# normallytangent/dune-eigensolver

Hardware: AMD Instinct MI355X
Metric: Lanczos iters/sec + achieved SpMV HBM GB/s, 3D Poisson 256^3 (higher is better)
Workload: dtype f64

## Files before the change

dune-eigensolver_amd/csrc/api.cpp:

```cpp
#include <algorithm>
#include <cmath>
#include <cstdlib>
#include <cstring>
#include <atomic>
#include <mutex>
#include <random>
#include <thread>

#include "internal.h"

using namespace eigmi;

namespace {

struct DeviceGuard {
  int prev = -1;
  explicit DeviceGuard(int dev)
  {
    if (hipGetDevice(&prev) != hipSuccess) prev = -1;
    if (prev != dev) EIG_HIP(hipSetDevice(dev));
  }
  ~DeviceGuard()
  {
    if (prev >= 0) (void)hipSetDevice(prev);
// ... 1628 lines not shown
    info->ncols = A->nb_cols * A->bc;
    info->row_begin = A->row_begin * A->br;
    info->window = A->window;
    info->own_offset = A->own_offset;
    info->nnzb = A->nnzb;
    info->nnzb_padded = A->nnzb_padded;
    info->nslices = A->nslices;
    info->br = A->br;
    info->bc = A->bc;
    info->halo_recv = A->halo_recv;
    info->halo_send = A->halo_send;
    info->device_bytes = A->device_bytes;
    info->stencil_slices = A->n_stencil_slices;
    info->rows_per_lane = A->R;
    info->sym_offsets = A->sym_val ? A->sym_nd : 0;
    info->sym_arrays = A->sym_val ? A->sym_nup : 0;
    info->sym_mask_bytes = A->sym_val ? A->sym_mask_bytes : 0;
    info->sym_uniform = (A->sym_val && A->sym_uniform && !(A->kflags & EIG_MAT_NO_UNIFORM))
                            ? (A->sym_geo ? 2 : 1)
                            : 0;
    info->sym_geo = A->sym_val && A->sym_geo ? 1 : 0;
    info->march_variant = march_variant(*A, true);
    info->march_variant_mv = march_variant(*A, false);
  });
}

extern "C" int eig_lanczos_kernel_info(eig_mat_t A, int fused, char *name, int name_len, int64_t *bytes)
{
  return guard(A ? A->ctx : nullptr, [&] {
    EIG_CHECK(A && bytes && (name || name_len == 0), EIG_ERR_ARG, "eig_lanczos_kernel_info: null argument");
    std::string nm;
    i64 b = 0;
    lanczos_kernel_info(*A, fused != 0, nm, b);
    *bytes = b;
    if (name_len > 0)
    {
      const size_t k = std::min<size_t>(nm.size(), (size_t)name_len - 1);
      std::memcpy(name, nm.data(), k);
      name[k] = 0;
    }
  });
}

extern "C" int eig_mat_kernel_info(eig_mat_t A, int op, char *name, int name_len)
{
  return guard(A ? A->ctx : nullptr, [&] {
// ... 549 lines not shown
```

dune-eigensolver_amd/csrc/drivers.cpp:

```cpp
#include <algorithm>
#include <complex>
#include <cmath>
#include <cstdlib>
#include <cstring>
#include <numeric>
#include <string>
#include <vector>

#include "internal.h"

using namespace eigmi;

namespace {

bool distributed(const eig_mat_s &A) { return A.ctx->distributed(); }

struct PinnedDoubles {
  double *p = nullptr, *dev = nullptr;
  explicit PinnedDoubles(size_t n)
  {
    EIG_HIP(hipHostMalloc(reinterpret_cast<void **>(&p), (n ? n : 1) * sizeof(double), hipHostMallocMapped));
    EIG_HIP(hipHostGetDevicePointer(reinterpret_cast<void **>(&dev), p, 0));
  }
  ~PinnedDoubles()
// ... 1686 lines not shown
      }
      launch_fused_tail(ws->lb->st, ws->L, ctx->stream);
    }
    else
      launch_beta_tail(ws->lb->st, ws->k, ctx->stream);
    EIG_HIP(hipStreamSynchronize(ctx->stream));
    check_step_exchange(*ws);
    if (k) *k = ws->k;
    if (alpha_host && ws->k > 0)
      EIG_HIP(hipMemcpy(alpha_host, ws->lb->st.alpha, ws->k * sizeof(double), hipMemcpyDeviceToHost));
    if (beta_host) EIG_HIP(hipMemcpy(beta_host, ws->lb->st.beta, (ws->k + 1) * sizeof(double), hipMemcpyDeviceToHost));
  });
}

extern "C" int eig_lanczos_info(eig_lanczos_t ws, int *steps, int *launches)
{
  return guard(ws ? ws->A->ctx : nullptr, [&] {
    EIG_CHECK(ws, EIG_ERR_ARG, "eig_lanczos_info: null workspace");
    if (steps) *steps = ws->k;
    if (launches) *launches = ws->fused ? ws->L : ws->k;
  });
}

extern "C" int eig_lanczos_destroy(eig_lanczos_t ws)
{
  if (!ws) return EIG_OK;
  (void)hipSetDevice(ws->A->ctx->device);
  (void)hipStreamSynchronize(ws->A->ctx->stream);
  delete ws;
  return EIG_OK;
}

extern "C" int eig_lanczos_run(eig_mat_t A, int steps, const double *u0, unsigned seed, int flags, double *alpha_host,
                               double *beta_host, eig_timing *timing)
{
  eig_lanczos_t ws = nullptr;
  const int kind = EIG_LANCZOS_FUSED | EIG_LANCZOS_PIPELINED;
  int rc = eig_lanczos_create_ex(A, steps, u0, seed, flags & kind, &ws);
  if (rc != EIG_OK) return rc;
  rc = eig_lanczos_step(ws, steps, flags & ~kind, timing);
  if (rc == EIG_OK) rc = eig_lanczos_tridiag(ws, nullptr, alpha_host, beta_host);
  eig_lanczos_destroy(ws);
  return rc;
}

extern "C" int eig_lanczos_solve(eig_mat_t A, int nev, int ncv, int which, unsigned seed, double *eval_host,
// ... 99 lines not shown
```

dune-eigensolver_amd/csrc/internal.h:

```cpp
#pragma once
#include <hip/hip_runtime.h>
#include <rccl/rccl.h>

#include <complex>
#include <condition_variable>
#include <cstdint>
#include <mutex>
#include <new>
#include <stdexcept>
#include <string>
#include <memory>
#include <vector>

#include "../../include/eigmi.h"

namespace eigmi {

typedef int64_t i64;
typedef int32_t i32;
typedef uint64_t u64;

struct Error : std::runtime_error {
  int code;
  Error(int c, const std::string &m) : std::runtime_error(m), code(c) {}
// ... 233 lines not shown
  double *fred;
  int *ctl;
  double *aux;
  double *mu2;
  double *pn;
};
enum { kFusedModeStep = 0, kFusedModePost = 1, kFusedModeHalt = 2 };
struct FusedLaunch {
  LanczosState st;
  int L;
  int force;
  int xch = 0;
};
enum { kXchPublish = 2 };
void launch_lanczos_fused(const eig_mat_s &A, const double *P, double *Pout, const FusedLaunch &fl,
                          const i32 *slices, i64 first, i64 count, const double *carry, double *out, int ticket,
                          hipStream_t s, ReduceWS red);
void launch_lanczos_pipe(const eig_mat_s &A, double *T, double *UZ, const double *S, const FusedLaunch &fl,
                         double *out, hipStream_t s, ReduceWS red);
void launch_fused_tail(const LanczosState &st, int L, hipStream_t s);
bool march_geometry(const eig_mat_s &A, i64 &D, int chunk = 64);
bool march_split_active(const eig_mat_s &A);
int march_variant(const eig_mat_s &A, bool fused);
extern const i32 kMarchInteriorTag;
bool box_prepare(const eig_mat_s &A);
inline bool box_spmm_applies(const eig_mat_s &A, i64 m)
{
  return m > 0 && m % 8 == 0 && box_prepare(A) && (A.box_ctab != nullptr || m % 32 == 0);
}
int box_cols(const eig_mat_s &A);
bool launch_box_spmm(const eig_mat_s &A, i64 m, const double *X, double *Y, hipStream_t s);
bool launch_box_spmm_dot(const eig_mat_s &A, i64 m, const double *X, double *Y, double *dp, ReduceWS red,
                         hipStream_t s);
bool launch_box_spmm_dot_gram(const eig_mat_s &A, i64 m, const double *X, double *Y, double *dp, double *gram,
                              ReduceWS red, hipStream_t s, unsigned *zero_word = nullptr);
bool launch_spmm_march_dot_gram(const eig_mat_s &A, i64 m, const double *X, double *Y, double *dp, double *gram,
                                ReduceWS red, hipStream_t s, unsigned *zero_word = nullptr);
unsigned *mgs_lookahead_barrier(eig_ctx_t ctx);
bool launch_spmm_dot_gram_mv8(const eig_mat_s &A, i64 m, const double *X, double *Y, double *dp, double *gram,
                              hipStream_t s, ReduceWS red);
bool launch_spmm_march_dot(const eig_mat_s &A, i64 m, const double *X, double *Y, double *dp, ReduceWS red,
                           hipStream_t s);
bool launch_box_cheb(const eig_mat_s &M, i64 m, const double *Xk, double *Xold, const double *B, const double *dinv,
                     double omega, double gamma, hipStream_t s, double *Xnew = nullptr);
void box_invalidate(eig_mat_s &A);
bool launch_box_resid(const eig_mat_s &A, i64 m, const double *X, const double *B, double *R, hipStream_t s);
// ... 217 lines not shown
```

dune-eigensolver_amd/csrc/k_spmv.hip:

```cpp
#include "internal.h"
#include "march_variants.h"
#include "reduce_dev.h"
#include "xch_dev.h"

namespace eigmi {

constexpr int kWaves = kStreamThreads / 64;

template <int R>
struct Vec;
template <>
struct Vec<1> {
  typedef double d;
  typedef i32 i;
};
template <>
struct Vec<2> {
  typedef double d __attribute__((ext_vector_type(2)));
  typedef i32 i __attribute__((ext_vector_type(2)));
};
template <>
struct Vec<4> {
  typedef double d __attribute__((ext_vector_type(4)));
  typedef i32 i __attribute__((ext_vector_type(4)));
};

// ... 1071 lines not shown
  }
  double v[3] = {d, q2, m2};
  fused_finish<2>(v, partials, ticket, tot, out, carry, fa);
}

struct MarchPlan {
  i64 D;
  i64 zb;
  i64 nplanes;
  i64 mrows;
  int ncol;
  int nseg;
  i32 dn, dq;
  const double *Un, *Uq;
  double cD, c0, c1, cn, cq;
  int gx, gy, gz, gz0;
  int uni;
  int tstore;
  signed char kj[27];
  const double *pack;
  int cache;
  int lines;
  int down;
};
template <class T>
__device__ __forceinline__ void march_store(const MarchPlan &mp, T v, T *p)
{
  if (mp.tstore)
    *p = v;
  else
    __builtin_nontemporal_store(v, p);
}

template <int PF, bool PG, class X, class EPI>
__device__ __forceinline__ void march_rows_geo(const SellB1 &A, const MarchPlan &mp, i64 own, int lane, int wave,
                                               const X &x, EPI &epi)
{
  typedef typename X::raw raw;
  const SymImg &S = A.sym;
  const int xl = (int)A.xlast, D = (int)mp.D, own32 = (int)own;
  const int nd = S.nd;
  const int item = (int)swizzled_block() * kWaves + wave;
  if (item >= mp.ncol * mp.nseg) return;
  const int col = item % mp.ncol, seg = item / mp.ncol;
  const int z0 = (int)(mp.zb + seg * mp.nplanes / mp.nseg), z1 = (int)(mp.zb + (seg + 1) * mp.nplanes / mp.nseg);
  auto cx = [&](int g) -> unsigned { return g < 0 ? 0u : (unsigned)(g > xl ? xl : g); };
// ... 251 lines not shown
  };
  static_assert(!PG || NS % 2 == 0, "gather prefetch: an even number of bodies per trip");
  static_assert(!VPF || NS % 2 == 0, "value prefetch: an even number of bodies per trip");
  int z = z0;
  for (; z + NS - 1 < z1; z += NS)
  {
#pragma unroll
    for (int k = 0; k < NS; ++k)
      body(z + k, sl[k], sl[(k + 1) % NS], sl[(k + PF + 1) % NS], gs[PG ? k & 1 : 0], gs[PG ? (k + 1) & 1 : 1],
           vs[VPF ? k & 1 : 0], vs[VPF ? (k + 1) & 1 : 1]);
  }
#pragma unroll
  for (int k = 0; k < NS - 1; ++k)
    if (z + k < z1)
      body(z + k, sl[k], sl[(k + 1) % NS], sl[(k + PF + 1) % NS], gs[PG ? k & 1 : 0], gs[PG ? (k + 1) & 1 : 1],
           vs[VPF ? k & 1 : 0], vs[VPF ? (k + 1) & 1 : 1]);
}

constexpr bool kMarch2lDefault = true;
constexpr bool kMarch2lSerpentine = true;
constexpr bool march_down_variant(int uni) { return uni == 22 || uni == 23; }
template <int UNI>
constexpr bool kMarchDownBody = march_down_variant(UNI);

template <bool DOWN, class X, class EPI, class PRE>
__device__ __forceinline__ void march_rows_geo2_2l(const SellB1 &A, const MarchPlan &mp, i64 own, int lane, int wave,
                                                   X x, EPI &epi, PRE &pre)
{
  typedef typename X::raw raw;
  constexpr unsigned SZ = sizeof(raw);
  const int D = (int)mp.D, own32 = (int)own, gx = mp.gx;
  const int item = (int)swizzled_block() * kWaves + wave;
  if (item >= mp.ncol * mp.nseg) return;
  const int col2 = item % mp.ncol, seg = item / mp.ncol;
  const int xcols = gx / 64;
  const int x0 = (col2 % xcols) * 64, y0 = (col2 / xcols) * 2;
  const int z0 = (int)(mp.zb + seg * mp.nplanes / mp.nseg), z1 = (int)(mp.zb + (seg + 1) * mp.nplanes / mp.nseg);
  const unsigned nbytes = (unsigned)(A.xlast + 1) * SZ;
  const __amdgpu_buffer_rsrc_t rs = __builtin_amdgcn_make_buffer_rsrc(const_cast<void *>(x.ptr()), 0, (int)nbytes, 0x00020000);
  const __amdgpu_buffer_rsrc_t r0 = __builtin_amdgcn_make_buffer_rsrc(const_cast<void *>(x.ptr()), 0, 0, 0x00020000);
  const bool has_n = mp.dn && y0 > 0, has_q = mp.dq && y0 + 2 < mp.gy;
  const __amdgpu_buffer_rsrc_t rn = has_n ? rs : r0, rq = has_q ? rs : r0;
  constexpr unsigned kOut = 0x80000000u;
  const unsigned eoff = lane == 0 ? (x0 > 0 ? 0u - SZ : kOut) : lane == 63 ? (x0 + 64 < gx ? SZ : kOut) : kOut;
  const unsigned dnb = (unsigned)mp.dn * SZ, dqb = (unsigned)mp.dq * SZ, Db = (unsigned)D * SZ, nxb = (unsigned)gx * SZ;
  int w = own32 + y0 * gx + x0 + lane + z0 * D;
  unsigned vo = (unsigned)w * SZ;
  const int zg0 = z0 + mp.gz0;
  const SymImg &S = A.sym;
  const dpair *P01 = reinterpret_cast<const dpair *>(mp.pack), *P23 = P01 + S.ld;
  const bool le = lane == 0 && x0 > 0;
  if constexpr (DOWN)
  {
    auto row = [&](double amD, double vmD, double an, double vn, double am, double vl, double a0, double vc, double a1,
                   double vr, double aq, double vq, double prodD) {
      double acc = 0.0;
      acc += amD * vmD;
      acc += an * vn;
      acc += am * vl;
      acc += a0 * vc;
      acc += a1 * vr;
      acc += aq * vq;
      acc += prodD;
      return acc;
    };
    w += (z1 - 1 - z0) * D;
    vo = (unsigned)w * SZ;
    const bool above = z1 + mp.gz0 < mp.gz;
    raw pu0{}, pu1{};
    if (above)
    {
      bload(rs, vo + Db, pu0);
      bload(rs, vo + nxb + Db, pu1);
    }
// ... 323 lines not shown

template <int UNI>
constexpr MarchTraits kTraits = march_traits(UNI);
template <int UNI>
constexpr bool kWholePlanes = kTraits<UNI>.whole_planes();
template <int UNI>
constexpr bool kUniformValues = kTraits<UNI>.values == kMarchUniform;

template <class MT, int KC, bool SPAN1, int UNI, class X, class EPI, class PRE = MarchNoPre>
__device__ __forceinline__ void march_rows(const SellB1 &A, const MarchPlan &mp, i64 own, int lane, int wave,
                                           const X &x, EPI &epi, PRE &&pre = PRE{})
{
  static_assert(kTraits<UNI>.valid, "not a march variant (march_variants.h)");
  static_assert(kTraits<UNI>.any_head() ||
                    (SPAN1 == kTraits<UNI>.span1() && (int)sizeof(MT) == kTraits<UNI>.mask_bytes()),
                "march variant instantiated with another template head than its traits name");
  if constexpr (kTraits<UNI>.family == kMarchKuhn)
  {
    march_rows_kuhn<kTraits<UNI>.kp, kTraits<UNI>.lx>(A, mp, own, lane, wave, x, epi, pre);
    return;
  }
  else if constexpr (kTraits<UNI>.family == kMarchGeo2L2)
  {
    if constexpr (kMarchDownBody<UNI>)
      if (mp.down)
      {
        march_rows_geo2_2l<true>(A, mp, own, lane, wave, x, epi, pre);
        return;
      }
    march_rows_geo2_2l<false>(A, mp, own, lane, wave, x, epi, pre);
    return;
  }
  else if constexpr (kTraits<UNI>.family == kMarchGeo2)
  {
    march_rows_geo2<kTraits<UNI>.pf, kTraits<UNI>.pg, kTraits<UNI>.val>(A, mp, own, lane, wave, x, epi, pre);
    return;
  }
  else if constexpr (kTraits<UNI>.family == kMarchGeo)
  {
    march_rows_geo<kTraits<UNI>.pf, kTraits<UNI>.pg>(A, mp, own, lane, wave, x, epi);
    return;
  }
  constexpr bool GEO = kTraits<UNI>.geo_masks;
  typedef typename X::raw raw;
  const SymImg &S = A.sym;
  const int xl = (int)A.xlast, D = (int)mp.D, ldl = (int)(S.ld - 1), own32 = (int)own, mrows = (int)mp.mrows;
// ... 815 lines not shown
    mp.gz = A.sym_gz;
    mp.gz0 = A.sym_gz0;
  }
  if (A.sym_uniform)
  {
    const int kD = A.sym_nd - 1;
    int kz = -1, k1 = -1;
    for (int k = 0; k < A.sym_nd; ++k)
    {
      if (A.sym_off[k] == 0) kz = k;
      if (A.sym_off[k] == 1) k1 = k;
    }
    mp.cD = A.sym_uc[A.sym_dj[kD]];
    mp.c0 = kz >= 0 ? A.sym_uc[A.sym_dj[kz]] : 0.0;
    mp.c1 = k1 >= 0 ? A.sym_uc[A.sym_dj[k1]] : 0.0;
    mp.cn = klo > 1 ? A.sym_uc[A.sym_dj[1]] : 0.0;
    mp.cq = khi < A.sym_nd - 1 ? A.sym_uc[A.sym_dj[khi]] : 0.0;
  }
  mp.uni = uni;
  mp.pack = pack && T.needs_pack() ? sym_pack_prepare(A) : nullptr;
  mp.tstore = fused && T.geo2_path() && (vectors_fit_mall(A) || (A.tune_cache & 1));
  mp.cache = A.tune_cache;
  mp.down = march_down_variant(uni) && (A.tune_cache & 24) == 16;
  mp.lines = A.tune_march_lines == 4 && T.line_groups && mp.gx % 64 == 0 &&
                     mp.gx > 0 && mp.gy % 4 == 0 && (i64)mp.gx * mp.gy == D
                 ? 4
                 : 0;
  mp.zb = zb;
  mp.nplanes = nplanes;
  mp.mrows = A.nslices * 64;
  mp.ncol = (int)items_per_run;
  mp.nseg = (int)nseg;
  return mp;
}

int march_variant(const eig_mat_s &A, bool fused)
{
  if (A.br != 1 || A.bc != 1) return -1;
  const MarchPlan mp = march_plan(A, image_mode(A), 0, -1, fused);
  return mp.nseg > 0 ? mp.uni : -1;
}

const i32 kMarchInteriorTag = 0;

void march_prepare(const eig_mat_s &A)
{
  if (A.br != 1 || A.bc != 1) return;
  const int mode = image_mode(A);
  for (bool fused : {false, true})
  {
    (void)march_plan(A, mode, 0, -1, fused, 64, true);
    if (A.mz1 > A.mz0) (void)march_plan(A, mode, A.mz0, A.mz1, fused, 64, true);
  }
}

bool march_split_active(const eig_mat_s &A)
{
  return A.mz1 > A.mz0 && march_plan(A, image_mode(A), A.mz0, A.mz1).nseg > 0;
}

static MarchPlan launch_plan(const eig_mat_s &A, int mode, const i32 *slices, i64 first, i64 count,
                             bool fused = false)
{
// ... 138 lines not shown
    fa.mb = A.ctx->mbox->dev;
  }
#define EIG_LFB(B_)                                                                                          \
  if (A.br == B_)                                                                                            \
  {                                                                                                          \
    hipLaunchKernelGGL((k_lanczos_fused_blk<B_>),                                                            \
                       dim3(grid_for_slices(k_lanczos_fused_blk<B_>, count, A.ctx->num_cu)),                 \
                       dim3(kStreamThreads), 0, s, A.nb_rows, A.slice_ptr, slices, first, count, A.val, A.col, \
                       reinterpret_cast<const dpair *>(P), reinterpret_cast<dpair *>(Pout), fa, out, carry,   \
                       red.partials, red.ticket(ticket));                                                    \
    return;                                                                                                  \
  }
  EIG_LFB(2) EIG_LFB(3) EIG_LFB(4)
#undef EIG_LFB
  if (!carry)
  {
    const int mode = image_mode(A);
    MarchPlan mp = launch_plan(A, mode, slices, first, count, true);
    if (mp.nseg > 0)
    {
      if (march_down_variant(mp.uni) && ((A.tune_cache & 24) == 24 || (kMarch2lSerpentine && !(A.tune_cache & 24))))
        mp.down = fl.L & 1;
      march_launch(MarchDispatch{}, A, mode, mp.uni, [&](auto mt, auto span1, auto uni) {
        hipLaunchKernelGGL((k_lanczos_fused_march<decltype(mt), span1(), uni()>), dim3(march_grid(mp)),
                           dim3(kStreamThreads), 0, s, A.nb_rows, A.own_offset, sell_b1(A), mp,
                           reinterpret_cast<const dpair *>(P), reinterpret_cast<dpair *>(Pout), fa, out, red.partials,
                           red.ticket(ticket));
      });
      return;
    }
  }
#define EIG_LF_(R_, M_, CPF_)                                                                                 \
  hipLaunchKernelGGL((k_lanczos_fused_b1<R_, M_, CPF_>),                                                     \
                     dim3(grid_for_slices(k_lanczos_fused_b1<R_, M_, CPF_>, count, A.ctx->num_cu)),           \
                     dim3(kStreamThreads), 0, s, A.nb_rows, A.own_offset, sell_b1(A), slices, first, count,      \
                     reinterpret_cast<const dpair *>(P), reinterpret_cast<dpair *>(Pout), fa, out, carry,        \
                     red.partials, red.ticket(ticket))
#define EIG_LF(R_, M_)                                                                                        \
  do                                                                                                          \
  {                                                                                                           \
    if (sell_cpf(A, true) && (M_ == kExplicit || M_ == kMixed)) EIG_LF_(R_, M_, true);                        \
    else EIG_LF_(R_, M_, false);                                                                              \
  } while (0)
#define EIG_LFM(R_)                                                                                           \
  {                                                                                                           \
    const int m_ = image_mode(A);                                                                             \
    if (m_ == kExplicit) EIG_LF(R_, kExplicit);                                                               \
    else if (m_ == kStencil) EIG_LF(R_, kStencil);                                                            \
// ... 242 lines not shown
```

dune-eigensolver_amd/eigmi.py:

```python
import atexit
import ctypes
import itertools
import os
import weakref

import numpy as np

_HERE = os.path.dirname(os.path.abspath(__file__))
LIB_PATH = os.path.join(_HERE, "lib", "libeigmi_san.so" if os.environ.get("EIGMI_LIB_VARIANT") == "san"
                        else "libeigmi.so")

EIG_OK, EIG_ERR_SHAPE, EIG_ERR_BLOCKSIZE, EIG_ERR_HIP, EIG_ERR_RCCL, EIG_ERR_BREAKDOWN, EIG_ERR_ARG, EIG_ERR_NODEVICE = range(8)
ORTHO_MGS, ORTHO_CHOLQR, ORTHO_CHOLQR_SPLIT = 0, 1, 2
ORTHO_GRID = 0x100
ORTHO_NO_COOP = 0x200
ORTHO_ONE_WG = 0x400


def ORTHO_LOOKAHEAD(L):
    return int(L) << 12

MAT_NO_BAND, MAT_BAND_GATHER, MAT_NO_STENCIL, MAT_NO_MARCH, MAT_NO_CLASS, MAT_NO_UNIFORM = 1, 2, 4, 8, 16, 32
TRSV_AUTO, TRSV_BLOCKINV, TRSV_STAGED, TRSV_CSR = 0, 1, 2, 3
TRSV_KINDS = {None: TRSV_AUTO, "auto": TRSV_AUTO, "blockinv": TRSV_BLOCKINV, "staged": TRSV_STAGED, "csr": TRSV_CSR}
# ... 18 lines not shown


GEN_LAPLACE2D, GEN_NEUMANN2D, GEN_PU2D, GEN_IDENTITY2D, GEN_POISSON3D, GEN_Q1ELAST3D, GEN_P1STIFF3D, GEN_P1MASS3D, \
    GEN_VARCOEF3D, GEN_P1STIFF3D_VAR, GEN_P1MASS3D_VAR = range(11)


class EigError(RuntimeError):
    def __init__(self, code, msg):
        super().__init__(f"[{code}] {msg}")
        self.code = code


class EigShapeError(EigError, ValueError):
    """SHAPE / BLOCKSIZE errors: the reference throws std::invalid_argument for these."""


class _MatInfo(ctypes.Structure):
    _fields_ = [(k, ctypes.c_int64) for k in ("n", "n_global", "ncols", "row_begin", "window", "own_offset", "nnzb",
                                              "nnzb_padded", "nslices")] + \
               [("br", ctypes.c_int), ("bc", ctypes.c_int)] + \
               [(k, ctypes.c_int64) for k in ("halo_recv", "halo_send", "device_bytes", "stencil_slices",
                                              "rows_per_lane", "sym_offsets", "sym_arrays",
                                              "sym_mask_bytes", "sym_uniform", "sym_geo",
                                              "march_variant", "march_variant_mv")]


class BlockTiming(ctypes.Structure):
    _fields_ = [(k, ctypes.c_double) for k in ("total_ms", "kspmm_ms", "cheb_ms", "orth_ms", "norm_ms")] + \
               [("steps", ctypes.c_int64), ("cheb_launches", ctypes.c_int64), ("cholqr_recomputed", ctypes.c_int64)]


class Timing(ctypes.Structure):
    _fields_ = [("total_ms", ctypes.c_double), ("spmv_ms", ctypes.c_double), ("update_ms", ctypes.c_double),
                ("comm_ms", ctypes.c_double), ("spmv_launches", ctypes.c_int64)]


_vp = ctypes.c_void_p
_i64 = ctypes.c_int64
_int = ctypes.c_int
_dbl = ctypes.c_double
_u = ctypes.c_uint

SIGNATURES = {
    "eig_ctx_create": (_int, [_int, ctypes.POINTER(_vp)]),
    "eig_ctx_destroy": (_int, [_vp]),
    "eig_last_error": (ctypes.c_char_p, [_vp]),
    "eig_ctx_sync": (_int, [_vp]),
# ... 54 lines not shown
    "eig_lanczos_update": (_int, [_vp, _i64, _vp, _vp, _vp, _vp, _vp, _vp]),
    "eig_spmm_dot_gram_mv8": (_int, [_vp, _i64, _vp, _vp, _vp, _vp]),
    "eig_orthonormalize_gram_mv8": (_int, [_vp, _i64, _i64, _vp, _vp]),
    "eig_stream_copy_timed": (_int, [_vp, _i64, _vp, _vp, _int, _int, ctypes.POINTER(_dbl)]),
    "eig_spmm_mv8": (_int, [_vp, _i64, _vp, _vp]),
    "eig_spmm_blk_mv8": (_int, [_vp, _i64, _vp, _vp]),
    "eig_dot_diag_mv8": (_int, [_vp, _i64, _i64, _vp, _vp, _vp]),
    "eig_gram_mv8": (_int, [_vp, _i64, _i64, _i64, _vp, _vp, _vp]),
    "eig_orthonormalize_mv8": (_int, [_vp, _i64, _i64, _vp, _int]),
    "eig_orthonormalize_passes": (_int, [_vp, ctypes.POINTER(ctypes.c_int)]),
    "eig_orthonormalize_naive": (_int, [_vp, _i64, _i64, _vp]),
    "eig_b_orthonormalize_mv8": (_int, [_vp, _i64, _vp, _vp]),
    "eig_random_mv8": (_int, [_vp, _i64, _i64, _u, _vp]),
    "eig_random_normal": (_int, [_i64, _u, _vp]),
    "eig_standard_largest": (_int, [_vp, _dbl, _dbl, _int, _int, _u, _vp, _vp, ctypes.POINTER(_int), _int]),
    "eig_lanczos_run": (_int, [_vp, _int, _vp, _u, _int, _vp, _vp, ctypes.POINTER(Timing)]),
    "eig_lanczos_solve": (_int, [_vp, _int, _int, _int, _u, _vp, _vp, _vp]),
    "eig_lanczos_create": (_int, [_vp, _int, _vp, _u, ctypes.POINTER(_vp)]),
    "eig_lanczos_create_ex": (_int, [_vp, _int, _vp, _u, _int, ctypes.POINTER(_vp)]),
    "eig_lanczos_step": (_int, [_vp, _int, _int, ctypes.POINTER(Timing)]),
    "eig_lanczos_tridiag": (_int, [_vp, ctypes.POINTER(_int), _vp, _vp]),
    "eig_lanczos_destroy": (_int, [_vp]),
    "eig_lanczos_info": (_int, [_vp, ctypes.POINTER(_int), ctypes.POINTER(_int)]),
    "eig_lanczos_capture": (_int, [_vp, _int, _int, ctypes.POINTER(_int)]),
    "eig_lanczos_ws_info": (_int, [_vp, ctypes.POINTER(_int), ctypes.c_char_p, _int, ctypes.POINTER(_i64)]),
    "eig_lanczos_replay": (_int, [_vp, ctypes.POINTER(Timing)]),
    "eig_lu_create": (_int, [_vp, _i64, _vp, _vp, _vp, _vp, _vp, _vp, _vp, _vp, _vp, _int, ctypes.POINTER(_vp)]),
    "eig_lu_create_bcsr": (_int, [_vp, _i64, _int, _vp, _vp, _vp, ctypes.POINTER(_vp)]),
    "eig_lu_info": (_int, [_vp, ctypes.POINTER(_i64), ctypes.POINTER(_i64), ctypes.POINTER(_i64), ctypes.POINTER(_int)]),
    "eig_lu_export": (_int, [_vp, _vp, _vp, _vp, _vp, _vp, _vp, _vp, _vp, _vp]),
    "eig_lu_destroy": (_int, [_vp]),
    "eig_inverse_mv8": (_int, [_vp, _i64, _vp, _vp]),
    "eig_standard_inverse": (_int, [_vp, _vp, _dbl, _dbl, _int, _int, _u, _vp, _vp, ctypes.POINTER(_int), _int]),
    "eig_generalized_inverse": (_int, [_vp, _vp, _vp, _dbl, _dbl, _dbl, _int, _int, _u, _vp, _vp, ctypes.POINTER(_int),
                                       _int]),
    "eig_shift_invert_solve": (_int, [_vp, _vp, _vp, _dbl, _int, _int, _dbl, _int, _u, _vp, _vp, ctypes.POINTER(_int)]),
    "eig_shift_invert_solve_ex": (_int, [_vp, _vp, _vp, _dbl, _int, _int, _dbl, _int, _u, _vp, _vp,
                                         ctypes.POINTER(_int), _int]),
    "eig_blanczos_create": (_int, [_vp, _vp, _int, _int, _int, _dbl, _dbl, _u, ctypes.POINTER(_vp)]),
    "eig_blanczos_create_si": (_int, [_vp, _vp, _vp, _dbl, _int, _int, _int, _dbl, _dbl, _u, ctypes.POINTER(_vp)]),
    "eig_blanczos_step": (_int, [_vp, _int, ctypes.POINTER(BlockTiming)]),
    "eig_mg_create": (_int, [_vp, _int, _int, _int, _int, _int, _dbl, ctypes.POINTER(_vp)]),
    "eig_mg_info": (_int, [_vp, ctypes.POINTER(_int), ctypes.POINTER(_i64), ctypes.POINTER(_int),
                           ctypes.POINTER(_dbl)]),
    "eig_mg_solve": (_int, [_vp, _i64, _vp, _vp, _int, ctypes.POINTER(_dbl)]),
    "eig_mg_destroy": (_int, [_vp]),
# ... 465 lines not shown
                name.value.decode(), b.value)

    def step(self, steps, timed=False):
        t = Timing()
        self.A.ctx.check(lib.eig_lanczos_step(self.h, steps, _tflags(timed), ctypes.byref(t)))
        return t

    def capture(self, steps, timed=False):
        c = _int(0)
        self.A.ctx.check(lib.eig_lanczos_capture(self.h, steps, _tflags(timed),
                                                 ctypes.byref(c)))
        return bool(c.value)

    def replay(self):
        t = Timing()
        self.A.ctx.check(lib.eig_lanczos_replay(self.h, ctypes.byref(t)))
        return t

    def info(self):
        k, L = _int(0), _int(0)
        self.A.ctx.check(lib.eig_lanczos_info(self.h, ctypes.byref(k), ctypes.byref(L)))
        return k.value, L.value

    def tridiag(self):
        k = _int(0)
        self.A.ctx.check(lib.eig_lanczos_tridiag(self.h, ctypes.byref(k), None, None))
        alpha = np.zeros(max(k.value, 1))
        beta = np.zeros(k.value + 1)
        self.A.ctx.check(lib.eig_lanczos_tridiag(self.h, ctypes.byref(k), _np_ptr(alpha), _np_ptr(beta)))
        return alpha[:k.value], beta

    def close(self):
        if self.h and self.A.h and self.A.ctx.h:
            lib.eig_lanczos_destroy(self.h)
        self.h = None

    def __del__(self):
        try:
            self.close()
        except Exception:
            pass


def lanczos_solve(A, nev, ncv, which=WHICH_LA, seed=123, want_evec=True):
    ev = np.zeros(nev)
    evec = np.zeros(nev * A.n) if want_evec else None
# ... 395 lines not shown
```

include/eigmi.h:

```cpp
#ifndef EIGMI_H
#define EIGMI_H

#include <stddef.h>
#include <stdint.h>

#ifdef __cplusplus
extern "C" {
#endif

#define EIGMI_VERSION_MAJOR 0
#define EIGMI_VERSION_MINOR 1

enum eig_status {
  EIG_OK = 0,
  EIG_ERR_SHAPE = 1,
  EIG_ERR_BLOCKSIZE = 2,
  EIG_ERR_HIP = 3,
  EIG_ERR_RCCL = 4,
  EIG_ERR_BREAKDOWN = 5,
  EIG_ERR_ARG = 6,
  EIG_ERR_NODEVICE = 7
};

typedef struct eig_ctx_s *eig_ctx_t;
// ... 62 lines not shown
typedef struct eig_mat_info {
  int64_t n;
  int64_t n_global;
  int64_t ncols;
  int64_t row_begin;
  int64_t window;
  int64_t own_offset;
  int64_t nnzb;
  int64_t nnzb_padded;
  int64_t nslices;
  int br, bc;
  int64_t halo_recv;
  int64_t halo_send;
  int64_t device_bytes;
  int64_t stencil_slices;
  int64_t rows_per_lane;
  int64_t sym_offsets;
  int64_t sym_arrays;
  int64_t sym_mask_bytes;
  int64_t sym_uniform;
  int64_t sym_geo;
  int64_t march_variant;
  int64_t march_variant_mv;
} eig_mat_info;
int eig_mat_get_info(eig_mat_t mat, eig_mat_info *info);

int eig_lanczos_kernel_info(eig_mat_t mat, int fused, char *name, int name_len, int64_t *bytes);
enum { EIG_OP_SPMV = 0, EIG_OP_LANCZOS_K1 = 1, EIG_OP_LANCZOS_FUSED = 2, EIG_OP_SPMM8 = 3, EIG_OP_CHEB8 = 4,
       EIG_OP_SPMM32 = 5, EIG_OP_CHEB32 = 6  };
int eig_mat_kernel_info(eig_mat_t mat, int op, char *name, int name_len);

enum { EIG_TUNE_MARCH_RUNS = 1, EIG_TUNE_BOX_SEGS = 2, EIG_TUNE_MARCH_PREFETCH = 3, EIG_TUNE_HALO = 4,
       EIG_TUNE_CACHE = 5, EIG_TUNE_BOX_COLS = 6, EIG_TUNE_BOX_MAP = 7, EIG_TUNE_SELL_CPF = 8,
       EIG_TUNE_MARCH_LINES = 9 };
#define EIG_MARCH_2L_MIN_ROWS 4194304
int eig_mat_tune(eig_mat_t mat, int key, int value);

int eig_mat_shift_diag(eig_mat_t mat, double shift);

int eig_mv(eig_mat_t mat, const double *x, double *y);
int eig_mv_host(eig_mat_t mat, const double *x_host, double *y_host);
int eig_mv_timed(eig_mat_t mat, const double *x, double *y, int reps, double *avg_ms);

int eig_dot(eig_ctx_t ctx, int64_t n, const double *x, const double *y, double *result);
int eig_nrm2(eig_ctx_t ctx, int64_t n, const double *x, double *result);
int eig_axpy(eig_ctx_t ctx, int64_t n, double a, const double *x, double *y);
int eig_scal(eig_ctx_t ctx, int64_t n, double a, double *x);
int eig_copy(eig_ctx_t ctx, int64_t n, const double *x, double *y);
int eig_lanczos_update(eig_ctx_t ctx, int64_t n, const double *alpha, const double *beta, const double *v,
                       const double *vprev, double *w, double *result);
int eig_stream_copy_timed(eig_ctx_t ctx, int64_t n, const double *x, double *y, int reps, int mode,
                          double *avg_ms);

int eig_spmm_mv8(eig_mat_t mat, int64_t m, const double *Qin, double *Qout);
int eig_spmm_blk_mv8(eig_mat_t mat, int64_t m, const double *Qin, double *Qout);
int eig_dot_diag_mv8(eig_ctx_t ctx, int64_t n, int64_t m, const double *Q1, const double *Q2, double *dp);
int eig_gram_mv8(eig_ctx_t ctx, int64_t n, int64_t m1, int64_t m2, const double *Q1, const double *Q2, double *G);
enum eig_ortho_variant { EIG_ORTHO_MGS = 0, EIG_ORTHO_CHOLQR = 1, EIG_ORTHO_CHOLQR_SPLIT = 2 };
// ... 20 lines not shown
  double spmv_ms;
  double update_ms;
  double comm_ms;
  int64_t spmv_launches;
} eig_timing;
enum eig_lanczos_flags {
  EIG_LANCZOS_TIME_KERNELS = 1,
  EIG_LANCZOS_TIME_DETAIL = 2,
  EIG_LANCZOS_FUSED = 4,
  EIG_LANCZOS_PIPELINED = 8,
  EIG_LANCZOS_AUTO = 16
};
int eig_lanczos_run(eig_mat_t A, int steps, const double *u0, unsigned seed, int flags,
                    double *alpha_host, double *beta_host, eig_timing *timing);

typedef struct eig_lanczos_s *eig_lanczos_t;
int eig_lanczos_create(eig_mat_t A, int max_steps, const double *u0, unsigned seed, eig_lanczos_t *ws);
int eig_lanczos_create_ex(eig_mat_t A, int max_steps, const double *u0, unsigned seed, int flags,
                          eig_lanczos_t *ws);
int eig_lanczos_step(eig_lanczos_t ws, int steps, int flags, eig_timing *timing);
int eig_lanczos_tridiag(eig_lanczos_t ws, int *k, double *alpha_host, double *beta_host);
int eig_lanczos_destroy(eig_lanczos_t ws);
int eig_lanczos_info(eig_lanczos_t ws, int *steps, int *launches);
int eig_lanczos_ws_info(eig_lanczos_t ws, int *variant, char *name, int name_len, int64_t *bytes);
int eig_lanczos_capture(eig_lanczos_t ws, int steps, int flags, int *captured);
int eig_lanczos_replay(eig_lanczos_t ws, eig_timing *timing);

enum eig_which { EIG_WHICH_LA = 0, EIG_WHICH_SA = 1 };
int eig_lanczos_solve(eig_mat_t A, int nev, int ncv, int which, unsigned seed, double *eval_host,
                      double *evec_host, double *resid_host);

typedef struct eig_lu_s *eig_lu_t;
int eig_lu_create(eig_ctx_t ctx, int64_t n, const int64_t *Lp, const int64_t *Lj, const double *Lx,
                  const int64_t *Up, const int64_t *Ui, const double *Ux, const int64_t *P, const int64_t *Q,
                  const double *Rs, int do_recip, eig_lu_t *lu);
int eig_lu_create_bcsr(eig_ctx_t ctx, int64_t nb_rows, int br, const int64_t *rowptr, const int32_t *col,
                       const double *vals, eig_lu_t *lu);
int eig_lu_info(eig_lu_t lu, int64_t *n, int64_t *lnz, int64_t *unz, int *do_recip);
enum { EIG_TRSV_AUTO = 0, EIG_TRSV_BLOCKINV = 1, EIG_TRSV_STAGED = 2, EIG_TRSV_CSR = 3 };
int eig_lu_set_solver(eig_lu_t lu, int kind);
int eig_lu_solver_info(eig_lu_t lu, int *kind, int *coupled_l, int *coupled_u);
int eig_lu_export(eig_lu_t lu, int64_t *Lp, int64_t *Lj, double *Lx, int64_t *Up, int64_t *Ui, double *Ux,
                  int64_t *P, int64_t *Q, double *Rs);
int eig_lu_destroy(eig_lu_t lu);
int eig_inverse_mv8(eig_lu_t lu, int64_t m, double *Qin, double *Qout);

// ... 81 lines not shown
```

Measured before the change: 5374.

## Add LDS double-buffered buffer-to-LDS prefetch pipeline for fused 2-layer march

Result: faster. 5642, median of 6 (+5.0%).

```diff
diff --git a/dune-eigensolver_amd/csrc/api.cpp b/dune-eigensolver_amd/csrc/api.cpp
--- a/dune-eigensolver_amd/csrc/api.cpp
+++ b/dune-eigensolver_amd/csrc/api.cpp
@@ -1674,6 +1674,7 @@
     info->sym_geo = A->sym_val && A->sym_geo ? 1 : 0;
     info->march_variant = march_variant(*A, true);
     info->march_variant_mv = march_variant(*A, false);
+    info->march_pipe = march_pipe(*A);
   });
 }
 
diff --git a/dune-eigensolver_amd/csrc/drivers.cpp b/dune-eigensolver_amd/csrc/drivers.cpp
--- a/dune-eigensolver_amd/csrc/drivers.cpp
+++ b/dune-eigensolver_amd/csrc/drivers.cpp
@@ -1732,6 +1732,21 @@
   });
 }
 
+extern "C" int eig_lanczos_pairs(eig_lanczos_t ws, double *pairs_host, int64_t rows)
+{
+  return guard(ws ? ws->A->ctx : nullptr, [&] {
+    EIG_CHECK(ws && pairs_host, EIG_ERR_ARG, "eig_lanczos_pairs: null argument");
+    EIG_CHECK(ws->fused && !ws->pipe, EIG_ERR_ARG, "eig_lanczos_pairs: the fused step's workspace only");
+    const eig_mat_s &A = *ws->A;
+    EIG_CHECK(A.br == 1 && A.bc == 1 && rows == A.nb_rows, EIG_ERR_SHAPE, "eig_lanczos_pairs: the owned rows of a 1x1 matrix");
+    eig_ctx_t ctx = A.ctx;
+    EIG_HIP(hipSetDevice(ctx->device));
+    EIG_HIP(hipStreamSynchronize(ctx->stream));
+    EIG_HIP(hipMemcpy(pairs_host, ws->B[ws->L & 1]->d() + 2 * A.own_offset, 2 * rows * sizeof(double),
+                      hipMemcpyDeviceToHost));
+  });
+}
+
 extern "C" int eig_lanczos_destroy(eig_lanczos_t ws)
 {
   if (!ws) return EIG_OK;
diff --git a/dune-eigensolver_amd/csrc/internal.h b/dune-eigensolver_amd/csrc/internal.h
--- a/dune-eigensolver_amd/csrc/internal.h
+++ b/dune-eigensolver_amd/csrc/internal.h
@@ -279,6 +279,7 @@
 bool march_geometry(const eig_mat_s &A, i64 &D, int chunk = 64);
 bool march_split_active(const eig_mat_s &A);
 int march_variant(const eig_mat_s &A, bool fused);
+int march_pipe(const eig_mat_s &A);
 extern const i32 kMarchInteriorTag;
 bool box_prepare(const eig_mat_s &A);
 inline bool box_spmm_applies(const eig_mat_s &A, i64 m)
diff --git a/dune-eigensolver_amd/csrc/k_spmv.hip b/dune-eigensolver_amd/csrc/k_spmv.hip
--- a/dune-eigensolver_amd/csrc/k_spmv.hip
+++ b/dune-eigensolver_amd/csrc/k_spmv.hip
@@ -2,6 +2,9 @@
 #include "march_variants.h"
 #include "reduce_dev.h"
 #include "xch_dev.h"
+
+#include <atomic>
+#include <type_traits>
 
 namespace eigmi {
 
@@ -1119,6 +1122,7 @@
   int cache;
   int lines;
   int down;
+  int pipe;
 };
 template <class T>
 __device__ __forceinline__ void march_store(const MarchPlan &mp, T v, T *p)
@@ -1416,8 +1420,48 @@
 constexpr bool march_down_variant(int uni) { return uni == 22 || uni == 23; }
 template <int UNI>
 constexpr bool kMarchDownBody = march_down_variant(UNI);
-
-template <bool DOWN, class X, class EPI, class PRE>
+constexpr bool march_pipe_variant(int uni) { return uni == 22 || uni == 23; }
+template <int UNI>
+constexpr bool kMarchPipeBody = march_pipe_variant(UNI);
+
+constexpr int kMarchPipeRegions = 13;
+constexpr unsigned kMarchPipeBuf = kMarchPipeRegions * 1024u;
+constexpr unsigned kMarchPipeLds = kWaves * 2 * kMarchPipeBuf;
+constexpr int kMaxPipeDevices = 64;
+typedef __attribute__((address_space(3))) char lds_char;
+template <int AUX>
+__device__ __forceinline__ void bdma(__amdgpu_buffer_rsrc_t r, unsigned off, lds_char *l)
+{
+  __builtin_amdgcn_raw_ptr_buffer_load_lds(r, l, 16, (int)off, 0, 0, AUX);
+}
+__device__ __forceinline__ void lds_read_near(unsigned a, dpair &r6, dpair &r7, dpair &r9, dpair &r10, double &y8,
+                                              double &x11, double &x12)
+{
+  asm volatile("ds_read_b128 %0, %7 offset:6144\n\tds_read_b128 %1, %7 offset:7168\n\t"
+               "ds_read_b128 %2, %7 offset:9216\n\tds_read_b128 %3, %7 offset:10240\n\t"
+               "ds_read_b64 %4, %7 offset:8200\n\tds_read_b64 %5, %7 offset:11264\n\t"
+               "ds_read_b64 %6, %7 offset:12288\n\ts_waitcnt lgkmcnt(0)"
+               : "=&v"(r6), "=&v"(r7), "=&v"(r9), "=&v"(r10), "=&v"(y8), "=&v"(x11), "=&v"(x12)
+               : "v"(a)
+               : "memory");
+}
+__device__ __forceinline__ void lds_read_mid(unsigned a, dpair &r4, dpair &r5, dpair &r0, dpair &r1)
+{
+  asm volatile("ds_read_b128 %0, %4 offset:4096\n\tds_read_b128 %1, %4 offset:5120\n\tds_read_b128 %2, %4\n\t"
+               "ds_read_b128 %3, %4 offset:1024\n\ts_waitcnt lgkmcnt(0)"
+               : "=&v"(r4), "=&v"(r5), "=&v"(r0), "=&v"(r1)
+               : "v"(a)
+               : "memory");
+}
+__device__ __forceinline__ void lds_read_far(unsigned a, dpair &r2, dpair &r3)
+{
+  asm volatile("ds_read_b128 %0, %2 offset:2048\n\tds_read_b128 %1, %2 offset:3072\n\ts_waitcnt lgkmcnt(0)"
+               : "=&v"(r2), "=&v"(r3)
+               : "v"(a)
+               : "memory");
+}
+
+template <bool DOWN, bool PIPE = false, class X, class EPI, class PRE>
 __device__ __forceinline__ void march_rows_geo2_2l(const SellB1 &A, const MarchPlan &mp, i64 own, int lane, int wave,
                                                    X x, EPI &epi, PRE &pre)
 {
@@ -1444,6 +1488,222 @@
   const SymImg &S = A.sym;
   const dpair *P01 = reinterpret_cast<const dpair *>(mp.pack), *P23 = P01 + S.ld;
   const bool le = lane == 0 && x0 > 0;
+  if constexpr (PIPE)
+  {
+    static_assert(SZ == sizeof(dpair), "the pipelined body marches the fused step's pair vector");
+    extern __shared__ char march_pipe_lds[];
+    lds_char *const Lw = (lds_char *)march_pipe_lds + (unsigned)wave * (2 * kMarchPipeBuf);
+    const unsigned ra0 = (unsigned)(size_t)Lw + (unsigned)lane * 16u;
+    const unsigned ldb = (unsigned)S.ld * 16u;
+    const __amdgpu_buffer_rsrc_t rp = __builtin_amdgcn_make_buffer_rsrc(const_cast<dpair *>(P01), 0, (int)(2u * ldb), 0x00020000);
+    const bool edge = lane == 0 || lane == 63;
+    const bool lok = x0 > 0;
+    const unsigned eo = lane == 0 ? (lok ? 0u - SZ : 0u) : (lane == 63 && x0 + 64 < gx ? SZ : 0u), lo = lok ? 0u - SZ : 0u;
+    const unsigned no = has_n ? dnb : 0u, qo = has_q ? dqb : 0u;
+    auto issue = [&](unsigned v, unsigned xfar, unsigned pfar, lds_char *L) {
+      bdma<0>(rs, v + xfar, L);
+      bdma<0>(rs, v + nxb + xfar, L + 1024);
+      if (mp.cache & 2)
+      {
+        bdma<0>(rp, v + pfar, L + 2 * 1024);
+        bdma<0>(rp, v + nxb + pfar, L + 3 * 1024);
+      }
+      else
+      {
+        bdma<2>(rp, v + pfar, L + 2 * 1024);
+        bdma<2>(rp, v + nxb + pfar, L + 3 * 1024);
+      }
+      bdma<0>(rp, v + ldb, L + 4 * 1024);
+      bdma<0>(rp, v + ldb + nxb, L + 5 * 1024);
+      bdma<0>(rs, v + no, L + 6 * 1024);
+      bdma<0>(rs, v + nxb + qo, L + 7 * 1024);
+      bdma<0>(rp, v + ldb + no, L + 8 * 1024);
+      if (edge)
+      {
+        bdma<0>(rs, v + eo, L + 9 * 1024);
+        bdma<0>(rs, v + nxb + eo, L + 10 * 1024);
+      }
+      if (lane == 0)
+      {
+        bdma<0>(rp, v + ldb + lo, L + 11 * 1024);
+        bdma<0>(rp, v + ldb + nxb + lo, L + 12 * 1024);
+      }
+    };
+    const dpair zero = dpair{0.0, 0.0};
+    auto eok = [&] {
+      unsigned t = eo;
+      asm volatile("" : "+v"(t));
+      return t != 0u;
+    };
+    auto nz = [](unsigned t) {
+      t = __builtin_amdgcn_readfirstlane(t);
+      asm volatile("" : "+s"(t));
+      return t != 0u;
+    };
+    unsigned bo = 0;
+    if constexpr (DOWN)
+    {
+      auto row = [&](double amD, double vmD, double an, double vn, double am, double vl, double a0, double vc, double a1,
+                     double vr, double aq, double vq, double prodD) {
+        double acc = 0.0;
+        acc += amD * vmD;
+        acc += an * vn;
+        acc += am * vl;
+        acc += a0 * vc;
+        acc += a1 * vr;
+        acc += aq * vq;
+        acc += prodD;
+        return acc;
+      };
+      w += (z1 - 1 - z0) * D;
+      vo = (unsigned)w * SZ;
+      const int gbot = -mp.gz0;
+      issue(vo, z1 - 1 > gbot ? 0u - Db : 0u, z1 - 1 > gbot ? 0u - Db : 0u, Lw);
+      const bool above = z1 + mp.gz0 < mp.gz;
+      raw pu0{}, pu1{};
+      if (above)
+      {
+        bload(rs, vo + Db, pu0);
+        bload(rs, vo + nxb + Db, pu1);
+      }
+      dpair p0a = (mp.cache & 2) ? P01[w] : __builtin_nontemporal_load(P01 + w);
+      dpair p1a = (mp.cache & 2) ? P01[w + gx] : __builtin_nontemporal_load(P01 + w + gx);
+      raw c0, c1;
+      bload(rs, vo, c0);
+      bload(rs, vo + nxb, c1);
+      const bool go = pre(x);
+      asm volatile("s_waitcnt vmcnt(0)" : "+v"(pu0), "+v"(pu1), "+v"(p0a), "+v"(p1a), "+v"(c0), "+v"(c1)::"memory");
+      if (!go) return;
+      double a00 = p0a.y, a01 = p1a.y;
+      double pD0 = p0a.x * (above ? x.val(pu0) : 0.0), pD1 = p1a.x * (above ? x.val(pu1) : 0.0);
+      for (int z = z1 - 1; z >= z0; --z)
+      {
+        if (z > z0)
+        {
+          const unsigned far = z - 1 > gbot ? 0u - Db : 0u;
+          issue(vo - Db, far, far, Lw + (bo ^ kMarchPipeBuf));
+          asm volatile("s_waitcnt vmcnt(15)" ::: "memory");
+        }
+        else
+          asm volatile("s_waitcnt vmcnt(2)" ::: "memory");
+        dpair m0, m1, q0a, q1a, p0b, p1b, xn0, xq1, eg0, eg1;
+        double any, ae0x, ae1x;
+        lds_read_near(ra0 + bo, xn0, xq1, eg0, eg1, any, ae0x, ae1x);
+        const bool hn = nz(no), lk = nz(lo);
+        if (!hn) xn0 = zero;
+        if (!nz(qo)) xq1 = zero;
+        if (!eok()) eg0 = eg1 = zero;
+        const double an0 = hn ? any : 0.0;
+        const double ae0 = lk ? ae0x : 0.0, ae1 = lk ? ae1x : 0.0;
+        double vn0 = x.val(xn0), vq1 = x.val(xq1), ve0 = x.val(eg0), ve1 = x.val(eg1);
+        asm volatile("" : "+v"(vn0), "+v"(vq1), "+v"(ve0), "+v"(ve1));
+        lds_read_mid(ra0 + bo, p0b, p1b, m0, m1);
+        lds_read_far(ra0 + bo, q0a, q1a);
+        if (!(z > gbot)) m0 = m1 = q0a = q1a = zero;
+        const double vc0 = x.val(c0), vc1 = x.val(c1);
+        const double acc0 = row(q0a.x, x.val(m0), an0, vn0, lane_shift_or<false>(p0b.x, ae0),
+                                lane_shift_or<false>(vc0, ve0), a00, vc0, p0b.x, lane_shift_or<true>(vc0, ve0), p0b.y,
+                                vc1, pD0);
+        const double acc1 = row(q1a.x, x.val(m1), p0b.y, vc0, lane_shift_or<false>(p1b.x, ae1),
+                                lane_shift_or<false>(vc1, ve1), a01, vc1, p1b.x, lane_shift_or<true>(vc1, ve1), p1b.y,
+                                vq1, pD1);
+        epi(w - own32, w, acc0, c0);
+        epi(w + gx - own32, w + gx, acc1, c1);
+        pD0 = q0a.x * vc0;
+        pD1 = q1a.x * vc1;
+        a00 = q0a.y;
+        a01 = q1a.y;
+        c0 = m0;
+        c1 = m1;
+        w -= D;
+        vo -= Db;
+        bo ^= kMarchPipeBuf;
+      }
+    }
+    else
+    {
+      const int gtop = mp.gz - 1 - mp.gz0;
+      issue(vo, z0 < gtop ? Db : 0u, 0u, Lw);
+      double amD0 = 0.0, amD1 = 0.0;
+      raw pm0{}, pm1{};
+      if (zg0 > 0)
+      {
+        bload(rs, vo - Db, pm0);
+        bload(rs, vo + nxb - Db, pm1);
+        amD0 = P01[w - D].x;
+        amD1 = P01[w + gx - D].x;
+      }
+      raw c0, c1;
+      bload(rs, vo, c0);
+      bload(rs, vo + nxb, c1);
+      const bool go = pre(x);
+      asm volatile("s_waitcnt vmcnt(0)" : "+v"(pm0), "+v"(pm1), "+v"(amD0), "+v"(amD1), "+v"(c0), "+v"(c1)::"memory");
+      if (!go) return;
+      double pmv0 = zg0 > 0 ? x.val(pm0) : 0.0, pmv1 = zg0 > 0 ? x.val(pm1) : 0.0;
+      for (int z = z0; z < z1; ++z)
+      {
+        if (z + 1 < z1)
+        {
+          issue(vo + Db, z + 1 < gtop ? Db : 0u, 0u, Lw + (bo ^ kMarchPipeBuf));
+          asm volatile("s_waitcnt vmcnt(15)" ::: "memory");
+        }
+        else
+          asm volatile("s_waitcnt vmcnt(2)" ::: "memory");
+        dpair d0, d1, p0a, p1a, p0b, p1b, xn0, xq1, eg0, eg1;
+        double any, ae0x, ae1x;
+        lds_read_near(ra0 + bo, xn0, xq1, eg0, eg1, any, ae0x, ae1x);
+        const bool hn = nz(no), lk = nz(lo);
+        if (!hn) xn0 = zero;
+        if (!nz(qo)) xq1 = zero;
+        if (!eok()) eg0 = eg1 = zero;
+        const double an0 = hn ? any : 0.0;
+        const double ae0 = lk ? ae0x : 0.0, ae1 = lk ? ae1x : 0.0;
+        double vn0 = x.val(xn0), vq1 = x.val(xq1), ve0 = x.val(eg0), ve1 = x.val(eg1);
+        asm volatile("" : "+v"(vn0), "+v"(vq1), "+v"(ve0), "+v"(ve1));
+        lds_read_mid(ra0 + bo, p0b, p1b, d0, d1);
+        lds_read_far(ra0 + bo, p0a, p1a);
+        if (!(z < gtop)) d0 = d1 = zero;
+        const double vc0 = x.val(c0), vc1 = x.val(c1);
+        double acc0 = 0.0, acc1 = 0.0;
+        {
+          const double ve = ve0;
+          const double vl = lane_shift_or<false>(vc0, ve), vr = lane_shift_or<true>(vc0, ve);
+          const double am = lane_shift_or<false>(p0b.x, ae0);
+          acc0 += amD0 * pmv0;
+          acc0 += an0 * vn0;
+          acc0 += am * vl;
+          acc0 += p0a.y * vc0;
+          acc0 += p0b.x * vr;
+          acc0 += p0b.y * vc1;
+          acc0 += p0a.x * x.val(d0);
+        }
+        {
+          const double ve = ve1;
+          const double vl = lane_shift_or<false>(vc1, ve), vr = lane_shift_or<true>(vc1, ve);
+          const double am = lane_shift_or<false>(p1b.x, ae1);
+          acc1 += amD1 * pmv1;
+          acc1 += p0b.y * vc0;
+          acc1 += am * vl;
+          acc1 += p1a.y * vc1;
+          acc1 += p1b.x * vr;
+          acc1 += p1b.y * vq1;
+          acc1 += p1a.x * x.val(d1);
+        }
+        epi(w - own32, w, acc0, c0);
+        epi(w + gx - own32, w + gx, acc1, c1);
+        pmv0 = vc0;
+        pmv1 = vc1;
+        amD0 = p0a.x;
+        amD1 = p1a.x;
+        c0 = d0;
+        c1 = d1;
+        w += D;
+        vo += Db;
+        bo ^= kMarchPipeBuf;
+      }
+    }
+    return;
+  }
   if constexpr (DOWN)
   {
     auto row = [&](double amD, double vmD, double an, double vn, double am, double vl, double a0, double vc, double a1,
@@ -1813,6 +2073,15 @@
   }
   else if constexpr (kTraits<UNI>.family == kMarchGeo2L2)
   {
+    if constexpr (kMarchPipeBody<UNI> && std::is_same<X, XPair>::value)
+      if (mp.pipe)
+      {
+        if (mp.down)
+          march_rows_geo2_2l<true, true>(A, mp, own, lane, wave, x, epi, pre);
+        else
+          march_rows_geo2_2l<false, true>(A, mp, own, lane, wave, x, epi, pre);
+        return;
+      }
     if constexpr (kMarchDownBody<UNI>)
       if (mp.down)
       {
@@ -2674,6 +2943,12 @@
   mp.tstore = fused && T.geo2_path() && (vectors_fit_mall(A) || (A.tune_cache & 1));
   mp.cache = A.tune_cache;
   mp.down = march_down_variant(uni) && (A.tune_cache & 24) == 16;
+  {
+    const i64 wgs = (items_per_run * nseg + kWaves - 1) / kWaves;
+    const bool can = fused && march_pipe_variant(uni) && A.sym_ld * 32 < (i64(1) << 32);
+    const bool pays = A.tune_march_prefetch != 0 || A.nb_rows >= EIG_MARCH_PIPE_MIN_ROWS;
+    mp.pipe = can && !(A.tune_cache & 32) && ((A.tune_cache & 64) || (wide_pack && wgs <= A.ctx->num_cu && pays));
+  }
   mp.lines = A.tune_march_lines == 4 && T.line_groups && mp.gx % 64 == 0 &&
                      mp.gx > 0 && mp.gy % 4 == 0 && (i64)mp.gx * mp.gy == D
                  ? 4
@@ -2691,6 +2966,13 @@
   if (A.br != 1 || A.bc != 1) return -1;
   const MarchPlan mp = march_plan(A, image_mode(A), 0, -1, fused);
   return mp.nseg > 0 ? mp.uni : -1;
+}
+
+int march_pipe(const eig_mat_s &A)
+{
+  if (A.br != 1 || A.bc != 1) return 0;
+  const MarchPlan mp = march_plan(A, image_mode(A), 0, -1, true);
+  return mp.nseg > 0 ? mp.pipe : 0;
 }
 
 const i32 kMarchInteriorTag = 0;
@@ -2875,8 +3157,23 @@
       if (march_down_variant(mp.uni) && ((A.tune_cache & 24) == 24 || (kMarch2lSerpentine && !(A.tune_cache & 24))))
         mp.down = fl.L & 1;
       march_launch(MarchDispatch{}, A, mode, mp.uni, [&](auto mt, auto span1, auto uni) {
+        if constexpr (march_pipe_variant(uni()))
+        {
+          static std::atomic<bool> raised[kMaxPipeDevices];
+          const int dev = A.ctx->device;
+          EIG_CHECK(!mp.pipe || (dev >= 0 && dev < kMaxPipeDevices), EIG_ERR_ARG, "pipelined march: device index");
+          if (mp.pipe && !raised[dev].load(std::memory_order_acquire))
+          {
+            EIG_HIP(hipFuncSetAttribute(
+                reinterpret_cast<const void *>(&k_lanczos_fused_march<decltype(mt), span1(), uni()>),
+                hipFuncAttributeMaxDynamicSharedMemorySize, (int)kMarchPipeLds));
+            raised[dev].store(true, std::memory_order_release);
+          }
+        }
+        else
+          mp.pipe = 0;
         hipLaunchKernelGGL((k_lanczos_fused_march<decltype(mt), span1(), uni()>), dim3(march_grid(mp)),
-                           dim3(kStreamThreads), 0, s, A.nb_rows, A.own_offset, sell_b1(A), mp,
+                           dim3(kStreamThreads), mp.pipe ? kMarchPipeLds : 0, s, A.nb_rows, A.own_offset, sell_b1(A), mp,
                            reinterpret_cast<const dpair *>(P), reinterpret_cast<dpair *>(Pout), fa, out, red.partials,
                            red.ticket(ticket));
       });
diff --git a/dune-eigensolver_amd/eigmi.py b/dune-eigensolver_amd/eigmi.py
--- a/dune-eigensolver_amd/eigmi.py
+++ b/dune-eigensolver_amd/eigmi.py
@@ -64,7 +64,7 @@
                [(k, ctypes.c_int64) for k in ("halo_recv", "halo_send", "device_bytes", "stencil_slices",
                                               "rows_per_lane", "sym_offsets", "sym_arrays",
                                               "sym_mask_bytes", "sym_uniform", "sym_geo",
-                                              "march_variant", "march_variant_mv")]
+                                              "march_variant", "march_variant_mv", "march_pipe")]
 
 
 class BlockTiming(ctypes.Structure):
@@ -165,6 +165,7 @@
     "eig_lanczos_tridiag": (_int, [_vp, ctypes.POINTER(_int), _vp, _vp]),
     "eig_lanczos_destroy": (_int, [_vp]),
     "eig_lanczos_info": (_int, [_vp, ctypes.POINTER(_int), ctypes.POINTER(_int)]),
+    "eig_lanczos_pairs": (_int, [_vp, _vp, _i64]),
     "eig_lanczos_capture": (_int, [_vp, _int, _int, ctypes.POINTER(_int)]),
     "eig_lanczos_ws_info": (_int, [_vp, ctypes.POINTER(_int), ctypes.c_char_p, _int, ctypes.POINTER(_i64)]),
     "eig_lanczos_replay": (_int, [_vp, ctypes.POINTER(Timing)]),
@@ -676,6 +677,11 @@
         self.A.ctx.check(lib.eig_lanczos_info(self.h, ctypes.byref(k), ctypes.byref(L)))
         return k.value, L.value
 
+    def pairs(self):
+        out = np.zeros((self.A.n, 2))
+        self.A.ctx.check(lib.eig_lanczos_pairs(self.h, _np_ptr(out), self.A.n))
+        return out
+
     def tridiag(self):
         k = _int(0)
         self.A.ctx.check(lib.eig_lanczos_tridiag(self.h, ctypes.byref(k), None, None))
diff --git a/include/eigmi.h b/include/eigmi.h
--- a/include/eigmi.h
+++ b/include/eigmi.h
@@ -108,6 +108,7 @@
   int64_t sym_geo;
   int64_t march_variant;
   int64_t march_variant_mv;
+  int64_t march_pipe;
 } eig_mat_info;
 int eig_mat_get_info(eig_mat_t mat, eig_mat_info *info);
 
@@ -120,6 +121,7 @@
        EIG_TUNE_CACHE = 5, EIG_TUNE_BOX_COLS = 6, EIG_TUNE_BOX_MAP = 7, EIG_TUNE_SELL_CPF = 8,
        EIG_TUNE_MARCH_LINES = 9 };
 #define EIG_MARCH_2L_MIN_ROWS 4194304
+#define EIG_MARCH_PIPE_MIN_ROWS 8388608
 int eig_mat_tune(eig_mat_t mat, int key, int value);
 
 int eig_mat_shift_diag(eig_mat_t mat, double shift);
@@ -186,6 +188,7 @@
 int eig_lanczos_tridiag(eig_lanczos_t ws, int *k, double *alpha_host, double *beta_host);
 int eig_lanczos_destroy(eig_lanczos_t ws);
 int eig_lanczos_info(eig_lanczos_t ws, int *steps, int *launches);
+int eig_lanczos_pairs(eig_lanczos_t ws, double *pairs_host, int64_t rows);
 int eig_lanczos_ws_info(eig_lanczos_t ws, int *variant, char *name, int name_len, int64_t *bytes);
 int eig_lanczos_capture(eig_lanczos_t ws, int steps, int flags, int *captured);
 int eig_lanczos_replay(eig_lanczos_t ws, eig_timing *timing);
```
